# SatDump/SatDump

Measured on AMD Instinct MI355X. Metric: Msamples/s IQ through PSK demod -> Viterbi -> RS (HBM-resident cf32), higher is better.
Workload: dtype f32; 1 GPU; metop_ahrpt (BASELINE configs[2]): QPSK 2333333 sym/s @ 6 Msps cf32, conv 3/4-metop, RS(255,223) I=4, 152880 CADUs = 2146959360 samples (17.176 GB) per GPU per step; mode=chunk-parallel (speculate + certify)

## Files before the change

satdump_amd/csrc/demod_kernels.hip:

```cpp
#include "demod_kernels.h"
#include <climits>
#include <optional>
#include <type_traits>

namespace sdhip
{
    static int env_int(const char *name, int dflt)
    {
        const char *v = getenv(name);
        return (v && *v) ? atoi(v) : dflt;
    }
    struct SinCosTab
    {
        double c0, c1, c2, c3, c4, s1, s2, s3;
    };
    __device__ __forceinline__ float sd_sinf_poly(double x, double x2, bool neg_tab, int n)
    {
        const double sgn = neg_tab ? -1.0 : 1.0;
        if ((n & 1) == 0)
        {
            const double s1c = -0x1.555545995a603p-3, s2c = 0x1.1107605230bc4p-7, s3c = -0x1.994eb3774cf24p-13;
            const double x3 = x * x2;
            const double s1 = fma(x2, s3c, s2c);
            const double x7 = x3 * x2;
// ... 42 lines not shown
        if (sd_abstop12(y) < sd_abstop12(0x1.921FB6p-1f))
        {
            if (sd_abstop12(y) < sd_abstop12(0x1p-12f))
                return 1.0f;
            return sd_sinf_poly(x, x * x, false, 1);
        }
        int n;
        x = sd_reduce_fast(x, &n);
        const double sgn = ((n & 3) == 1 || (n & 3) == 2) ? -1.0 : 1.0;
        return sd_sinf_poly(x * sgn, x * x, (n & 2) != 0, n ^ 1);
    }

    __device__ __forceinline__ void sd_sincosf(float y, float &sn, float &cs)
    {
        const double x0 = (double)y;
        int n;
        const double xr = sd_reduce_fast(x0, &n);
        const double xs = ((n + 1) & 2) ? -xr : xr;
        const double x2 = xr * xr;
        const double s1c = -0x1.555545995a603p-3, s2c = 0x1.1107605230bc4p-7, s3c = -0x1.994eb3774cf24p-13;
        const double x3 = xs * x2;
        const double s1 = fma(x2, s3c, s2c);
        const double x7 = x3 * x2;
        const double sp = fma(x7, s1, fma(x3, s1c, xs));
        const double c1c = -0x1.ffffffd0c621cp-2, c2c = 0x1.55553e1068f19p-5, c3c = -0x1.6c087e89a359dp-10, c4c = 0x1.99343027bf8c3p-16;
        const double x4 = x2 * x2;
        const double c2 = fma(x2, c4c, c3c);
        const double c1 = fma(x2, c1c, 0x1p0);
        const double x6 = x4 * x2;
        const double cp0 = fma(x6, c2, fma(x4, c2c, c1));
        const float fs = (float)sp, fc0 = (float)cp0;
        const float fc = (n & 2) ? -fc0 : fc0;
        const bool odd = (n & 1) != 0;
        const bool tiny = sd_abstop12(y) < sd_abstop12(0x1p-12f);
        sn = tiny ? y : (odd ? fc : fs);
        cs = tiny ? 1.0f : (odd ? fs : fc);
    }

    __device__ __forceinline__ void sd_sincosf_fast(float y, float &sn, float &cs)
    {
        const float k = rintf(y * 0.63661977236758134308f);
        float r = fmaf(-k, 1.57079637050628662109375f, y);
        r = fmaf(-k, -4.37113900018624283e-8f, r);
        const float r2 = r * r;
        const float sp = fmaf(r2, fmaf(r2, fmaf(r2, 2.75573192239858906526e-6f, -1.98412698412698412698e-4f), 8.33333333333333333333e-3f), -1.66666666666666666667e-1f);
        const float s = fmaf(r * r2, sp, r);
        const float cp = fmaf(r2, fmaf(r2, fmaf(r2, 2.48015873015873015873e-5f, -1.38888888888888888889e-3f), 4.16666666666666666667e-2f), -0.5f);
        const float c = fmaf(r2, cp, 1.0f);
        const int q = (int)k & 3;
        const float a = (q & 1) ? c : s, b = (q & 1) ? s : c;
        sn = (q & 2) ? -a : a;
        cs = ((q + 1) & 2) ? -b : b;
    }
    __device__ __forceinline__ float sd_sqrt_fast(float x)
    {
#ifdef SDHIP_HOST_TWIN
        return sqrtf(x);
#else
        return __builtin_amdgcn_sqrtf(x);
#endif
    }
    __device__ __forceinline__ float sd_clip_med3(float x, float lo, float hi)
    {
#ifdef SDHIP_HOST_TWIN
        return x != x ? lo : x < lo ? lo : (x > hi ? hi : x);
#else
        return __builtin_amdgcn_fmed3f(x, lo, hi);
#endif
    }

    __global__ __launch_bounds__(256) void k_convert(const void *in, int fmt, int iq_swap, long long n, cf32 *out)
    {
        const long long i = (long long)blockIdx.x * blockDim.x + threadIdx.x;
        if (i >= n)
            return;
        float re, im;
        if (fmt == 0)
        {
            const cf32 v = ((const cf32 *)in)[i];
            re = v.re;
            im = v.im;
        }
        else if (fmt == 1)
        {
            const short2 v = ((const short2 *)in)[i];
            const float s = 1.0f / 32767.0f;
            re = (float)v.x * s;
            im = (float)v.y * s;
        }
        else if (fmt == 2)
        {
            const char2 v = ((const char2 *)in)[i];
            const float s = 1.0f / 127.0f;
            re = (float)v.x * s;
            im = (float)v.y * s;
        }
        else if (fmt == 3)
        {
            const uchar2 v = ((const uchar2 *)in)[i];
            re = (float)((double)((int)v.x - 127) * (1.0 / 127.0));
            im = (float)((double)((int)v.y - 127) * (1.0 / 127.0));
        }
        else
        {
            const int2 v = ((const int2 *)in)[i];
            const float sc = 1.0f / 2147483647.0f;
// ... 564 lines not shown
            int z = 0;
            asm volatile("" : "+s"(z));
#pragma unroll
            for (int j = 0; j < NT; j++)
            {
                const float tk = rtaps[z + j];
                const v2f tt{tk, tk};
#pragma unroll
                for (int r = 0; r < FIRW_R; r++)
                {
                    const v2f prod = s[r + j] * tt;
                    acc[r] = acc[r] + prod;
                }
            }
#pragma unroll
            for (int r = 0; r < FIRW_R; r++)
                tile[t * FIRW_R + r] = acc[r];
            __syncthreads();
            const long long i0 = blk * OUTS;
            for (int i = t; i < OUTS; i += FIRW_BLOCK)
                if (i0 + i < n)
                    reinterpret_cast<v2f *>(y)[i0 + i] = tile[i];
            __syncthreads();
        }
    }
    static bool fir_window_enabled()
    {
        static const bool on = [] {
            const char *e = getenv("SDHIP_FIR_WINDOW");
            return !(e && e[0] == '0');
        }();
        return on;
    }
    void launch_fir(const cf32 *x, cf32 *y, long long n, const float *rtaps_dev, int ntaps, hipStream_t st)
    {
        if (n <= 0)
            return;
        if (ntaps == 31 && fir_window_enabled())
        {
            ProfScope _ps("k_fir_window", st);
            const long long ntiles = (n + FIRW_BLOCK * FIRW_R - 1) / (FIRW_BLOCK * FIRW_R);
            static const int grid = resident_grid(k_fir_window<31>, FIRW_BLOCK);
            hipLaunchKernelGGL((k_fir_window<31>), dim3((unsigned)(ntiles < grid ? ntiles : grid)), dim3(FIRW_BLOCK), 0, st, x, y, n, rtaps_dev, ntiles);
            return;
        }
        ProfScope _ps("k_fir", st);
        hipLaunchKernelGGL(k_fir, dim3((unsigned)((n + FIR_BLOCK * FIR_PER - 1) / (FIR_BLOCK * FIR_PER))), dim3(FIR_BLOCK), 0, st, x, y, n, rtaps_dev, ntaps);
    }

    struct Blk8
    {
        float4 a, b, c, d;
    };
    template <int D, bool FASTQ = false>
    struct AgcStageT
    {
        using P = AgcParams;
        using S = AgcState;
        static constexpr int DEPTH = D;
        __device__ static __forceinline__ S init(const P &p, int k) { return S{p.starts ? p.starts[k] : p.init_gain}; }
        __device__ static __forceinline__ bool close(const S &a, const S &b, float tol_a, float) { return fabsf(a.gain - b.gain) <= tol_a * fabsf(b.gain); }
        __device__ static __forceinline__ void prewarm(S &, const P &, const cf32 *, long long) {}
        __device__ static __forceinline__ cf32 step(S &s, const P &p, const cf32 v) { return step_t<FASTQ>(s, p, v); }
        template <bool FAST>
        __device__ static __forceinline__ cf32 step_t(S &s, const P &p, const cf32 v)
        {
            const float ore = v.re * s.gain;
            const float oim = v.im * s.gain;
            float mag;
            if (p.input_mag)
            {
                float mi;
                if constexpr (FAST)
                    mi = sd_sqrt_fast(fmaf(v.re, v.re, v.im * v.im));
                else
                    mi = sqrtf(v.re * v.re + v.im * v.im);
                mag = mi * s.gain;
            }
            else if constexpr (FAST)
                mag = sd_sqrt_fast(fmaf(ore, ore, oim * oim));
            else
                mag = sqrtf(ore * ore + oim * oim) ;
            s.gain = s.gain + p.rate * (p.reference - mag);
            if (p.max_gain > 0.0f && s.gain > p.max_gain)
                s.gain = p.max_gain;
            return cf32{ore, oim};
        }
    };

    using AgcStage = AgcStageT<4>;

    __device__ __forceinline__ float sd_to_vgpr(float v)
    {
        float r;
        asm("v_mov_b32 %0, %1" : "=v"(r) : "s"(v));
        return r;
    }
    template <bool FAST>
    struct AgcFirStageT
    {
        using P = AgcFirParams;
        using S = AgcFirState;
        static constexpr int DEPTH = 4;
        static constexpr int NT = AGCFIR_NT;
        __device__ static __forceinline__ S init(const P &p, int)
        {
            S s;
            s.gain = p.agc.init_gain;
#pragma unroll
            for (int i = 0; i < 4; i++)
                s.lag[i] = p.agc.init_gain;
#pragma unroll
            for (int i = 0; i < 2 * (NT - 1); i++)
                s.w[i] = 0.0f;
            return s;
        }
        __device__ static __forceinline__ bool close(const S &a, const S &b, float tol_a, float) { return fabsf(a.gain - b.gain) <= tol_a * fabsf(b.gain); }
        __device__ static __forceinline__ void prewarm(S &, const P &, const cf32 *, long long) {}
        __device__ static __forceinline__ v2f agc(S &s, const P &p, float re, float im)
        {
            AgcState a{s.gain};
            const cf32 o = AgcStageT<4>::template step_t<FAST>(a, p.agc, cf32{re, im});
            s.gain = a.gain;
            return v2f{o.re, o.im};
        }
        __device__ static __forceinline__ Blk8 block(S &s, const P &p, const Blk8 &c, bool write)
        {
            v2f loc[NT - 1 + 8];
#pragma unroll
            for (int i = 0; i < NT - 1; i++)
                loc[i] = v2f{s.w[2 * i], s.w[2 * i + 1]};
            const float g_in = s.gain;
            loc[NT - 1 + 0] = agc(s, p, c.a.x, c.a.y);
            loc[NT - 1 + 1] = agc(s, p, c.a.z, c.a.w);
            loc[NT - 1 + 2] = agc(s, p, c.b.x, c.b.y);
            loc[NT - 1 + 3] = agc(s, p, c.b.z, c.b.w);
            loc[NT - 1 + 4] = agc(s, p, c.c.x, c.c.y);
            loc[NT - 1 + 5] = agc(s, p, c.c.z, c.c.w);
            loc[NT - 1 + 6] = agc(s, p, c.d.x, c.d.y);
            loc[NT - 1 + 7] = agc(s, p, c.d.z, c.d.w);
            Blk8 o{};
            if (write)
            {
                v2f acc[8];
#pragma unroll
                for (int r = 0; r < 8; r++)
                    acc[r] = v2f{0.0f, 0.0f};
#pragma unroll
                for (int j = 0; j < NT; j++)
                {
                    const v2f tp{sd_to_vgpr(p.taps[j & ~1]), sd_to_vgpr(p.taps[j | 1])};
                    const v2f tt = (j & 1) ? __builtin_shufflevector(tp, tp, 1, 1) : __builtin_shufflevector(tp, tp, 0, 0);
                    if constexpr (FAST)
                    {
#pragma unroll
                        for (int r = 0; r < 8; r++)
                            acc[r] = __builtin_elementwise_fma(loc[r + j], tt, acc[r]);
                    }
                    else
                    {
                        v2f prod[8];
#pragma unroll
                        for (int r = 0; r < 8; r++)
                            prod[r] = loc[r + j] * tt;
#pragma unroll
                        for (int r = 0; r < 8; r++)
                            acc[r] = acc[r] + prod[r];
                    }
                }
                o = Blk8{make_float4(acc[0].x, acc[0].y, acc[1].x, acc[1].y), make_float4(acc[2].x, acc[2].y, acc[3].x, acc[3].y),
                         make_float4(acc[4].x, acc[4].y, acc[5].x, acc[5].y), make_float4(acc[6].x, acc[6].y, acc[7].x, acc[7].y)};
            }
#pragma unroll
            for (int i = 0; i < NT - 1; i++)
            {
                s.w[2 * i] = loc[i + 8].x;
                s.w[2 * i + 1] = loc[i + 8].y;
            }
            s.lag[3] = s.lag[2];
            s.lag[2] = s.lag[1];
            s.lag[1] = s.lag[0];
            s.lag[0] = g_in;
            return o;
        }
        __device__ static __forceinline__ cf32 step(S &s, const P &p, const cf32 v)
        {
            const v2f a = agc(s, p, v.re, v.im);
            v2f acc{0.0f, 0.0f};
#pragma unroll
            for (int j = 0; j < NT - 1; j++)
            {
                const v2f prod = v2f{s.w[2 * j], s.w[2 * j + 1]} * v2f{p.taps[j], p.taps[j]};
                acc = acc + prod;
            }
            {
                const v2f prod = a * v2f{p.taps[NT - 1], p.taps[NT - 1]};
                acc = acc + prod;
            }
#pragma unroll
            for (int i = 0; i < NT - 2; i++)
            {
                s.w[2 * i] = s.w[2 * i + 2];
                s.w[2 * i + 1] = s.w[2 * i + 3];
            }
            s.w[2 * (NT - 2)] = a.x;
            s.w[2 * (NT - 2) + 1] = a.y;
            return cf32{acc.x, acc.y};
        }
    };
    using AgcFirStage = AgcFirStageT<false>;

    template <int ORDER, int D = 4, bool FAST = false, bool BCLIP = false>
    struct CostasStage
    {
        using P = CostasParams;
        using S = CostasState;
        static constexpr int DEPTH = D;
        __device__ static __forceinline__ S init(const P &p, int) { return S{0.0f, p.init_freq}; }
        __device__ static __forceinline__ bool close(const S &a, const S &b, float tol_phase, float tol_freq)
        {
            const float twopi = 6.28318530717958647692f;
            float d = a.phase - b.phase;
            d -= twopi * rintf(d / twopi);
            return fabsf(d) < tol_phase && fabsf(a.freq - b.freq) < tol_freq;
        }
        __device__ static __forceinline__ void prewarm(S &s, const P &p, const cf32 *x, long long i0)
        {
            if (p.est_len <= 0 || p.order > 4)
                return;
            const int M = p.order;
            float rc, rs;
            __sincosf(-(float)M * s.freq, &rs, &rc);
            float cr = 1.0f, ci = 0.0f, ar = 0.0f, ai = 0.0f;
            for (int n = 0; n < p.est_len; n++)
            {
                const cf32 v = x[i0 + n];
                float zr = v.re * v.re - v.im * v.im, zi = 2.0f * v.re * v.im;
                if (M == 4)
                {
                    const float tr = zr * zr - zi * zi, ti = 2.0f * zr * zi;
                    zr = tr;
                    zi = ti;
                }
                ar += zr * cr - zi * ci;
                ai += zr * ci + zi * cr;
                const float nr = cr * rc - ci * rs, ni = cr * rs + ci * rc;
                cr = nr;
                ci = ni;
            }
            const float ang = (M == 4) ? atan2f(-ai, -ar) : atan2f(ai, ar);
            s.phase = ang / (float)M;
        }
        __device__ static __forceinline__ cf32 step(S &s, const P &p, const cf32 v)
        {
            float cs, sn;
            if constexpr (FAST)
                sd_sincosf_fast(-s.phase, sn, cs);
            else
                sd_sincosf(-s.phase, sn, cs);
            const float tr = (v.re * cs) - (v.im * sn);
            const float ti = (v.im * cs) + (v.re * sn);
            float error;
            if constexpr (ORDER == 2)
                error = tr * ti;
            else if constexpr (ORDER == 4)
                error = (tr > 0.0f ? 1.0f : -1.0f) * ti - (ti > 0.0f ? 1.0f : -1.0f) * tr;
            else
            {
                const float K = sqrtf(2.0f) - 1.0f;
                const float st = tr > 0.0f ? 1.0f : -1.0f, su = ti > 0.0f ? 1.0f : -1.0f;
                const float ea = st * ti - su * tr * K, eb = st * ti * K - su * tr;
                error = fabsf(tr) >= fabsf(ti) ? ea : eb;
            }
            if constexpr (BCLIP)
                error = error < -1.0f ? -1.0f : (error > 1.0f ? 1.0f : error);
            else
                error = 0.5f * (fabsf(error + 1.0f) - fabsf(error - 1.0f));
            s.freq = s.freq + p.beta * error;
            s.phase = s.phase + (s.freq + p.alpha * error);
            const double twopi = 2 * 3.14159265358979323846;
            {
                const float twopi_f = 6.28318548202514648f;
                const double step = s.phase >= twopi_f ? -twopi : (s.phase <= -twopi_f ? twopi : 0.0);
                s.phase = (float)((double)s.phase + step);
            }
            s.freq = __builtin_fmaxf(__builtin_fminf(s.freq, p.fmax), p.fmin);
            return cf32{tr, ti};
        }
    };

    __device__ __forceinline__ float sd_fast_atan2f(float y, float x, const float *__restrict__ tab)
    {
        const float ya = fabsf(y), xa = fabsf(x);
        if (!(ya > 0.0f || xa > 0.0f))
            return 0.0f;
        const bool flat = ya < xa;
        const float z = flat ? ya / xa : xa / ya;
        float base = z;
        if (!((double)z < 0.003921569))
        {
            const float al = z * 255.0f;
            const int idx = ((int)al) & 0xff;
            const float lo = tab[idx], hi = tab[idx + 1];
            base = lo + (hi - lo) * (al - (float)idx);
        }
        const float pi = (float)3.14159265358979323846, half = (float)1.57079632679489661923;
        if (xa > ya)
            return x >= 0.0f ? (y >= 0.0f ? base : -base) : (y >= 0.0f ? pi - base : base - pi);
        return y >= 0.0f ? (x >= 0.0f ? half - base : half + base) : (x >= 0.0f ? -half + base : -half - base);
    }
    __device__ __forceinline__ float sd_fast_cos(float x)
    {
        const float x2 = x * x, x4 = x2 * x2, x8 = x4 * x4;
        return (float)((-2.7236370439787708e-7 * x2 + 2.4799852696610628e-5) * x8 + (-1.3888885054799695e-3 * x2 + 4.1666666636943683e-2) * x4 +
                       (-4.9999999999963024e-1 * x2 + 1.0000000000000000e+0));
    }
    __device__ __forceinline__ float sd_fast_sin(float x)
    {
        const float x2 = x * x, x4 = x2 * x2;
        return (float)(((2.7181216275479732e-6 * x2 - 1.9839312269456257e-4) * x4 + (8.3333293048425631e-3 * x2 - 1.6666666640797048e-1)) * x2 * x + x);
    }
    __device__ __forceinline__ float sd_wrap_pi(float v)
    {
        const double pi = 3.14159265358979323846, twopi = 2 * 3.14159265358979323846;
        while ((double)v < -pi)
            v = (float)((double)v + twopi);
        while ((double)v > pi)
            v = (float)((double)v - twopi);
        return v;
    }
    struct PllStage
    {
        using P = PllParams;
        using S = CostasState;
        static constexpr int DEPTH = 2;
        __device__ static __forceinline__ S init(const P &p, int) { return S{0.0f, p.init_freq}; }
// ... 100 lines not shown
                s.fre_im *= inv;
                s.margin = fminf(s.margin, fminf(p.fmax - s.freq, s.freq - p.fmin));
                if (s.freq > p.fmax)
                {
                    s.freq = p.fmax;
                    s.fre_re = p.lim_min_re;
                    s.fre_im = p.lim_min_im;
                }
                if (s.freq < p.fmin)
                {
                    s.freq = p.fmin;
                    s.fre_re = p.lim_max_re;
                    s.fre_im = p.lim_max_im;
                }
            }
            return cf32{tr, ti};
        }
    };

    struct DcStage
    {
        using P = DcParams;
        using S = DcState;
        static constexpr int DEPTH = 4;
        __device__ static __forceinline__ S init(const P &p, int k) { return p.starts[k]; }
        __device__ static __forceinline__ bool close(const S &a, const S &b, float tol, float)
        {
            const float m = fmaxf(fabsf(b.acc_re), fabsf(b.acc_im));
            return fabsf(a.acc_re - b.acc_re) <= tol * m && fabsf(a.acc_im - b.acc_im) <= tol * m;
        }
        __device__ static __forceinline__ void prewarm(S &, const P &, const cf32 *, long long) {}
        __device__ static __forceinline__ cf32 step(S &s, const P &, const cf32 v)
        {
            const float alpha = 0.0001f, beta = 1.0f - 0.0001f;
            s.acc_re = s.acc_re * beta + v.re * alpha;
            s.acc_im = s.acc_im * beta + v.im * alpha;
            return cf32{v.re - s.acc_re, v.im - s.acc_im};
        }
    };

    __device__ __forceinline__ Blk8 blk_load(const cf32 *x, long long i)
    {
        const float4 *xp = reinterpret_cast<const float4 *>(x + i);
        return Blk8{xp[0], xp[1], xp[2], xp[3]};
    }
    template <class Stage, class = void>
    struct stage_is_blockwise : std::false_type
    {
    };
    template <class Stage>
    struct stage_is_blockwise<Stage, std::void_t<decltype(&Stage::block)>> : std::true_type
    {
    };
    template <class Stage>
    __device__ __forceinline__ Blk8 blk_step(typename Stage::S &s, const typename Stage::P &p, const Blk8 &c, bool write)
    {
        if constexpr (stage_is_blockwise<Stage>::value)
            return Stage::block(s, p, c, write);
        else
        {
            const cf32 a0 = Stage::step(s, p, cf32{c.a.x, c.a.y});
            const cf32 a1 = Stage::step(s, p, cf32{c.a.z, c.a.w});
            const cf32 a2 = Stage::step(s, p, cf32{c.b.x, c.b.y});
            const cf32 a3 = Stage::step(s, p, cf32{c.b.z, c.b.w});
            const cf32 a4 = Stage::step(s, p, cf32{c.c.x, c.c.y});
            const cf32 a5 = Stage::step(s, p, cf32{c.c.z, c.c.w});
            const cf32 a6 = Stage::step(s, p, cf32{c.d.x, c.d.y});
            const cf32 a7 = Stage::step(s, p, cf32{c.d.z, c.d.w});
            return Blk8{make_float4(a0.re, a0.im, a1.re, a1.im), make_float4(a2.re, a2.im, a3.re, a3.im), make_float4(a4.re, a4.im, a5.re, a5.im),
                        make_float4(a6.re, a6.im, a7.re, a7.im)};
        }
    }
    template <class Stage, int D>
    __device__ __forceinline__ void group_run(typename Stage::S &s, const typename Stage::P &p, const Blk8 (&q)[D], cf32 *y, long long i, bool write)
    {
        Blk8 o[D];
#pragma unroll
        for (int d = 0; d < D; d++)
            o[d] = blk_step<Stage>(s, p, q[d], write);
        if (write)
        {
            float4 *yp = reinterpret_cast<float4 *>(y + i);
#pragma unroll
            for (int d = 0; d < D; d++)
            {
                yp[4 * d + 0] = o[d].a;
                yp[4 * d + 1] = o[d].b;
                yp[4 * d + 2] = o[d].c;
                yp[4 * d + 3] = o[d].d;
            }
        }
    }
    struct NoHook
    {
        __device__ __forceinline__ bool operator()(long long) const { return false; }
    };
    template <class Stage, bool HOOK = false, class Hook = NoHook>
    __device__ __forceinline__ void run_range(typename Stage::S &s, const typename Stage::P &p, const cf32 *x, cf32 *y, long long i0, long long i1, bool write,
                                              long long hb = 0, int hstep = 0, Hook hook = Hook())
    {
        constexpr int D = Stage::DEPTH;
        long long i = i0;
        for (; i < i1 && (i & 7); i++)
        {
            const cf32 o = Stage::step(s, p, x[i]);
            if (write)
                y[i] = o;
        }
        if (i + 8 * D <= i1)
        {
            Blk8 qa[D], qb[D];
#pragma unroll
            for (int d = 0; d < D; d++)
                qa[d] = blk_load(x, i + 8 * d);
            for (;;)
            {
                const bool more_b = i + 16 * D <= i1;
                if (more_b)
                {
#pragma unroll
                    for (int d = 0; d < D; d++)
                        qb[d] = blk_load(x, i + 8 * (D + d));
                }
                group_run<Stage, D>(s, p, qa, y, i, write);
// ... 88 lines not shown
        return b;
    }
    __device__ __forceinline__ void coop_unpack(const Burst &b, const Coop &co, Blk8 &q0, Blk8 &q1)
    {
        __builtin_amdgcn_sched_barrier(0);
        *reinterpret_cast<float4 *>(co.lw + 0 * 8 * COOP_REGION) = b.c0;
        *reinterpret_cast<float4 *>(co.lw + 1 * 8 * COOP_REGION) = b.c1;
        *reinterpret_cast<float4 *>(co.lw + 2 * 8 * COOP_REGION) = b.c2;
        *reinterpret_cast<float4 *>(co.lw + 3 * 8 * COOP_REGION) = b.c3;
        *reinterpret_cast<float4 *>(co.lw + 4 * 8 * COOP_REGION) = b.c4;
        *reinterpret_cast<float4 *>(co.lw + 5 * 8 * COOP_REGION) = b.c5;
        *reinterpret_cast<float4 *>(co.lw + 6 * 8 * COOP_REGION) = b.c6;
        *reinterpret_cast<float4 *>(co.lw + 7 * 8 * COOP_REGION) = b.c7;
        sd_wave_sync();
        const float4 *r = reinterpret_cast<const float4 *>(co.lr);
        q0 = Blk8{r[0], r[1], r[2], r[3]};
        q1 = Blk8{r[4], r[5], r[6], r[7]};
        sd_wave_sync();
        __builtin_amdgcn_sched_barrier(0);
    }
    __device__ __forceinline__ void coop_store_half(const Blk8 &o, int half, const Coop &co)
    {
        float4 *w = reinterpret_cast<float4 *>(co.sw + half * 64);
        w[0] = o.a;
        w[1] = o.b;
        w[2] = o.c;
        w[3] = o.d;
    }
    __device__ __forceinline__ void coop_store_flush(cf32 *y, long long i0w, const Coop &co)
    {
        __builtin_amdgcn_sched_barrier(0);
        sd_wave_sync();
        char *sb = reinterpret_cast<char *>(y + i0w);
#pragma unroll
        for (int j = 0; j < 8; j++)
            *reinterpret_cast<float4 *>(sb + (long long)(8 * j) * co.stride + co.voff) = *reinterpret_cast<const float4 *>(co.sr + j * 8 * COOP_REGION);
        sd_wave_sync();
        __builtin_amdgcn_sched_barrier(0);
    }
    template <class Stage, bool COOP = false, class Hook>
    __device__ __forceinline__ void run_range1(typename Stage::S &s, const typename Stage::P &p, const cf32 *x, cf32 *y, long long i0, long long i1,
                                               long long write_from, long long hb, int hstep, Hook hook, const Coop *co = nullptr)
    {
        static_assert(Stage::DEPTH == 4, "four-block groups");
        long long i = i0;
        for (; i < i1 && (i & 7); i++)
        {
            const cf32 o = Stage::step(s, p, x[i]);
            if (i >= write_from)
                y[i] = o;
        }
        if (i + 32 <= i1)
        {
            if constexpr (COOP)
            {
                const long long lim = 1ll << 30;
                const long long wf = write_from - i, tl = i1 - i;
                const int total = sd_uniform((int)(tl < lim ? tl : lim));
                const int wfrom = sd_uniform((int)(wf < -lim ? -lim : (wf < lim ? wf : lim)));
                const int hoff = sd_uniform((int)((i - hb) & (long long)(hstep - 1)));
                const long long iw = sd_uniform(i);
                const long long ibase = i;
                int r = 0;
                Burst b0 = coop_load(x, iw, *co), b1 = coop_load(x, iw + 16, *co);
                Blk8 q[4];
                for (;;)
                {
                    const bool more = r + 64 <= total;
                    const bool wr = r >= wfrom;
                    coop_unpack(b0, *co, q[0], q[1]);
#pragma unroll
                    for (int d = 0; d < 2; d++)
                    {
                        const Blk8 o = blk_step<Stage>(s, p, q[d], wr);
                        if (wr)
                            coop_store_half(o, d, *co);
                    }
                    if (wr)
                        coop_store_flush(y, iw + r, *co);
                    if (more)
                        b0 = coop_load(x, iw + r + 32, *co);
                    coop_unpack(b1, *co, q[2], q[3]);
#pragma unroll
                    for (int d = 2; d < 4; d++)
                    {
                        const Blk8 o = blk_step<Stage>(s, p, q[d], wr);
                        if (wr)
                            coop_store_half(o, d - 2, *co);
                    }
                    if (wr)
                        coop_store_flush(y, iw + r + 16, *co);
                    if (more)
                        b1 = coop_load(x, iw + r + 48, *co);
                    r += 32;
                    if ((((r + hoff) & (hstep - 1)) == 0) && r < total)
                        (void)hook(ibase + r);
                    if (!more)
                        break;
                }
                i = ibase + r;
            }
            else
            {
            Blk8 q[4];
#pragma unroll
            for (int d = 0; d < 4; d++)
                q[d] = blk_load(x, i + 8 * d);
            for (;;)
            {
                const bool more = i + 64 <= i1;
                const bool wr = i >= write_from;
#pragma unroll
                for (int d = 0; d < 4; d++)
                {
                    const Blk8 o = blk_step<Stage>(s, p, q[d], wr);
                    if (wr)
                        blk_store<Stage>(y, i + 8 * d, o);
                    if ((d & 1) && more)
                    {
                        q[d - 1] = blk_load(x, i + 32 + 8 * (d - 1));
                        q[d] = blk_load(x, i + 32 + 8 * d);
                    }
                }
                i += 32;
                if ((((i - hb) & (long long)(hstep - 1)) == 0) && i < i1 && hook(i))
                    return;
                if (!more)
                    break;
            }
            }
        }
        for (; i < i1; i++)
        {
            const cf32 o = Stage::step(s, p, x[i]);
            if (i >= write_from)
                y[i] = o;
        }
    }

    template <class Stage, bool CKPT>
    __global__ __launch_bounds__(64) void k_chunks(const cf32 *x, cf32 *y, ChunkGeom g, typename Stage::P p, const typename Stage::S *start0,
                                                   typename Stage::S *spec, typename Stage::S *endst, const int *redo, int nredo, typename Stage::S *ck,
                                                   int ck_per_chunk, int ck_len, float tol_a, float tol_b, unsigned long long *ck_work)
    {
        const int idx = (int)(blockIdx.x * blockDim.x + threadIdx.x);
        int k;
        typename Stage::S s;
        if (redo)
        {
            if (idx >= nredo)
                return;
            k = redo[idx];
            s = spec[k];
        }
        else
        {
            k = idx;
            if (k >= g.K)
                return;
            if (k == 0)
                s = *start0;
            else
            {
                s = Stage::init(p, k);
                const long long b = chunk_begin(g, k);
                Stage::prewarm(s, p, x, b - g.W);
                run_range<Stage>(s, p, x, y, b - g.W, b, false);
                spec[k] = s;
            }
        }
        const long long b = chunk_begin(g, k), e = chunk_end(g, k);
        if constexpr (!CKPT)
        {
            run_range<Stage>(s, p, x, y, b, e, true);
            endst[k] = s;
        }
        else
        {
            bool merged = false;
            int jmax = 0;
            typename Stage::S *cks = ck + (size_t)k * ck_per_chunk;
            run_range<Stage, true>(s, p, x, y, b, e, true, b, ck_len, [&](long long i) -> bool {
                const int j = (int)((i - b) / ck_len) - 1;
                if (j < 0 || j >= ck_per_chunk)
                    return false;
                jmax = j + 1;
                if (redo && Stage::close(s, cks[j], tol_a, tol_b))
                {
                    merged = true;
                    return true;
                }
                cks[j] = s;
                return false;
            });
            if (!merged)
                endst[k] = s;
            if (redo && ck_work)
            {
                atomicAdd(ck_work, 1ull);
                atomicAdd(ck_work + 1, (unsigned long long)(jmax + 1));
                atomicAdd(ck_work + 2, (unsigned long long)((e - b + ck_len - 1) / ck_len));
            }
        }
    }

    template <bool FAST>
    struct AfcAgcOnly
    {
        using P = AfcParams;
        using S = AfcState;
        static constexpr int DEPTH = 4;
        __device__ static __forceinline__ Blk8 block(S &s, const P &p, const Blk8 &c, bool) { return AgcFirStageT<FAST>::block(s.af, p.af, c, false); }
        __device__ static __forceinline__ cf32 step(S &s, const P &p, const cf32 v) { return AgcFirStageT<FAST>::step(s.af, p.af, v); }
    };
    struct AfcEstState
    {
        AfcState s;
        float cr, ci, ar, ai, rc, rs;
    };
    template <int M, bool FAST>
    struct AfcEst
    {
        using P = AfcParams;
        using S = AfcEstState;
        static constexpr int DEPTH = 4;
        __device__ static __forceinline__ void acc(S &e, float re, float im)
        {
            float zr = re * re - im * im, zi = 2.0f * re * im;
            if constexpr (M == 4)
            {
                const float tr = zr * zr - zi * zi, ti = 2.0f * zr * zi;
                zr = tr;
                zi = ti;
            }
            e.ar += zr * e.cr - zi * e.ci;
            e.ai += zr * e.ci + zi * e.cr;
            const float nr = e.cr * e.rc - e.ci * e.rs, ni = e.cr * e.rs + e.ci * e.rc;
            e.cr = nr;
            e.ci = ni;
        }
        __device__ static __forceinline__ Blk8 block(S &e, const P &p, const Blk8 &c, bool)
        {
            const Blk8 f = AgcFirStageT<FAST>::block(e.s.af, p.af, c, true);
            acc(e, f.a.x, f.a.y);
            acc(e, f.a.z, f.a.w);
            acc(e, f.b.x, f.b.y);
            acc(e, f.b.z, f.b.w);
            acc(e, f.c.x, f.c.y);
            acc(e, f.c.z, f.c.w);
            acc(e, f.d.x, f.d.y);
            acc(e, f.d.z, f.d.w);
            return f;
        }
        __device__ static __forceinline__ cf32 step(S &e, const P &p, const cf32 v)
        {
            const cf32 f = AgcFirStageT<FAST>::step(e.s.af, p.af, v);
            acc(e, f.re, f.im);
            return f;
        }
    };
    template <int ORDER, bool FAST>
    struct AfcFull
    {
        using P = AfcParams;
        using S = AfcState;
        using Cos = CostasStage<ORDER, 4, FAST>;
        static constexpr int DEPTH = 4;
        __device__ static __forceinline__ Blk8 block(S &s, const P &p, const Blk8 &c, bool)
        {
            const Blk8 f = AgcFirStageT<FAST>::block(s.af, p.af, c, true);
            const cf32 a0 = Cos::step(s.cos, p.cos, cf32{f.a.x, f.a.y});
            const cf32 a1 = Cos::step(s.cos, p.cos, cf32{f.a.z, f.a.w});
            const cf32 a2 = Cos::step(s.cos, p.cos, cf32{f.b.x, f.b.y});
            const cf32 a3 = Cos::step(s.cos, p.cos, cf32{f.b.z, f.b.w});
            const cf32 a4 = Cos::step(s.cos, p.cos, cf32{f.c.x, f.c.y});
            const cf32 a5 = Cos::step(s.cos, p.cos, cf32{f.c.z, f.c.w});
            const cf32 a6 = Cos::step(s.cos, p.cos, cf32{f.d.x, f.d.y});
            const cf32 a7 = Cos::step(s.cos, p.cos, cf32{f.d.z, f.d.w});
            return Blk8{make_float4(a0.re, a0.im, a1.re, a1.im), make_float4(a2.re, a2.im, a3.re, a3.im), make_float4(a4.re, a4.im, a5.re, a5.im),
                        make_float4(a6.re, a6.im, a7.re, a7.im)};
        }
        __device__ static __forceinline__ cf32 step(S &s, const P &p, const cf32 v) { return Cos::step(s.cos, p.cos, AgcFirStageT<FAST>::step(s.af, p.af, v)); }
    };
    __device__ __forceinline__ float sd_wrap_2pi(double ph)
    {
        const double twopi = 2 * 3.14159265358979323846;
        while (ph > twopi)
            ph -= twopi;
        while (ph < -twopi)
            ph += twopi;
        return (float)ph;
    }
    template <int ORDER, bool FAST>
    __global__ __launch_bounds__(64) __attribute__((amdgpu_waves_per_eu(2, 2))) void k_afc(const cf32 *x, cf32 *y, ChunkGeom g, AfcParams p, const AfcState *start0, AfcState *spec, AfcState *endst,
                                                const int *redo, int nredo, AfcCkpt *ck, int ck_per_chunk, int ck_len, float tol_phase, float tol_freq, int coop_nb)
    {
        __shared__ __attribute__((aligned(16))) char coop_lds[2 * COOP_LDS_BYTES];
        const int idx = (int)(blockIdx.x * blockDim.x + threadIdx.x);
        const bool coop = !redo && coop_nb > 0 && (int)blockIdx.x < coop_nb;
        const Coop co = coop_make(coop_lds, (long long)g.L * (long long)sizeof(cf32));
        int k;
        AfcState s;
        bool leave_spec = false;
        long long i0;
        if (redo)
        {
            if (idx >= nredo)
                return;
            k = redo[idx];
            s = spec[k];
            i0 = chunk_begin(g, k);
        }
        else
        {
            if (coop_nb > 0)
            {
                if (coop)
                    k = 1 + idx;
                else
                {
                    const int j = ((int)blockIdx.x - coop_nb) * 8 + (int)threadIdx.x;
                    if ((int)threadIdx.x >= 8 || j >= g.K - 64 * coop_nb)
                        return;
                    k = j == 0 ? 0 : 64 * coop_nb + j;
                }
            }
            else
            {
                k = idx;
                if (k >= g.K)
                    return;
            }
            i0 = 0;
            s = *start0;
            const long long b = chunk_begin(g, k);
            const long long w0 = b - g.W - p.w_agc;
            if (k > 0)
                leave_spec = true;
            if (k > 0 && w0 > 0)
            {
                const auto nohook = [](long long) { return false; };
                const long long never = 1ll << 62;
                s.af = AgcFirStage::init(p.af, k);
                s.cos = CostasState{0.0f, p.cos.init_freq};
                if (coop)
                    run_range1<AfcAgcOnly<FAST>, true>(s, p, x, y, w0, b - g.W, never, 0, 1 << 30, nohook, &co);
                else
                    run_range1<AfcAgcOnly<FAST>>(s, p, x, y, w0, b - g.W, never, 0, 1 << 30, nohook);
                i0 = b - g.W;
                if (p.cos.est_len > 0 && ORDER <= 4)
                {
                    constexpr int M = ORDER <= 2 ? 2 : 4;
                    AfcEstState e;
                    e.s = s;
                    __sincosf(-(float)M * s.cos.freq, &e.rs, &e.rc);
                    e.cr = 1.0f;
                    e.ci = 0.0f;
                    e.ar = 0.0f;
                    e.ai = 0.0f;
                    if (coop)
                        run_range1<AfcEst<M, FAST>, true>(e, p, x, y, i0, i0 + p.cos.est_len, never, 0, 1 << 30, nohook, &co);
                    else
                        run_range1<AfcEst<M, FAST>>(e, p, x, y, i0, i0 + p.cos.est_len, never, 0, 1 << 30, nohook);
                    s = e.s;
                    const float ang = (M == 4) ? atan2f(-e.ai, -e.ar) : atan2f(e.ai, e.ar);
                    s.cos.phase = sd_wrap_2pi((double)(ang / (float)M) + (double)s.cos.freq * (double)p.cos.est_len);
                    i0 += p.cos.est_len;
                }
            }
        }
        const long long b = chunk_begin(g, k), e = chunk_end(g, k);
        bool merged = false;
        AfcCkpt *cks = ck ? ck + (size_t)k * ck_per_chunk : nullptr;
        const auto hook = [&](long long i) -> bool {
            if (i < b)
                return false;
            if (i == b)
            {
                if (leave_spec)
                    spec[k] = s;
                return false;
            }
            const int j = (int)((i - b) / ck_len) - 1;
            if (!cks || j >= ck_per_chunk)
                return false;
            if (redo)
            {
                const AfcCkpt o = cks[j];
                if (__float_as_uint(o.gain) == __float_as_uint(s.af.gain) && __float_as_uint(o.lag3) == __float_as_uint(s.af.lag[3]) &&
                    CostasStage<ORDER, 4>::close(s.cos, CostasState{o.phase, o.freq}, tol_phase, tol_freq))
                {
                    merged = true;
                    return true;
                }
            }
            cks[j] = AfcCkpt{s.af.gain, s.af.lag[3], s.cos.phase, s.cos.freq};
            return false;
        };
        if (coop)
            run_range1<AfcFull<ORDER, FAST>, true>(s, p, x, y, i0, e, b, b, ck_len, hook, &co);
        else
            run_range1<AfcFull<ORDER, FAST>>(s, p, x, y, i0, e, b, b, ck_len, hook);
        if (!merged)
            endst[k] = s;
    }
    void launch_afc(const cf32 *x, cf32 *y, const ChunkGeom &g, const AfcParams &p, const AfcState *start0, AfcState *spec, AfcState *endst, const int *redo,
                    int nredo, hipStream_t st, const AfcCkptCfg &ck, bool fast)
    {
        const int n = redo ? nredo : g.K;
        if (n <= 0)
            return;
        ProfScope _ps("k_afc", st);
        std::optional<ProfScope> _pr;
        if (redo)
            _pr.emplace("k_afc (re-run launches, included in k_afc)", st);
        auto go = [&](auto order, auto fm) {
            constexpr int O = decltype(order)::value;
            constexpr bool F = decltype(fm)::value;
            const bool coop_env = env_int("SDHIP_COOP", 1) != 0;
            int coop_nb = 0;
            if (coop_env && !redo && g.L % 16 == 0 && g.W % 16 == 0 && p.w_agc % 16 == 0 && p.cos.est_len % 16 == 0 && (long long)g.L > (long long)p.w_agc && g.K >= 66)
                coop_nb = (g.K - 2) / 64;
            const int nblk = coop_nb > 0 ? coop_nb + (g.K - 64 * coop_nb + 7) / 8 : (n + 63) / 64;
            if (!redo && coop_nb == 0 && g.K >= 66 && getenv("SDHIP_COOP_REQUIRE"))
                throw HipError("k_afc: cooperative access asked for (SDHIP_COOP_REQUIRE) but the geometry does not allow it");
            if (getenv("SDHIP_DEBUG") && !redo)
                fprintf(stderr, "[sdhip] k_afc: K %d L %d W %d w_agc %d est %d -> %d cooperative blocks of %d\n", g.K, g.L, g.W, p.w_agc, p.cos.est_len, coop_nb, nblk);
            hipLaunchKernelGGL((k_afc<O, F>), dim3(nblk), dim3(64), 0, st, x, y, g, p, start0, spec, endst, redo, nredo, ck.ck, ck.per_chunk,
                               ck.len > 0 ? ck.len : 2048, ck.tol_phase, ck.tol_freq, coop_nb);
        };
        auto by_order = [&](auto fm) {
            if (p.cos.order == 2)
                go(std::integral_constant<int, 2>{}, fm);
            else if (p.cos.order == 4)
                go(std::integral_constant<int, 4>{}, fm);
            else
                go(std::integral_constant<int, 8>{}, fm);
        };
        if (fast)
            by_order(std::true_type{});
        else
            by_order(std::false_type{});
    }

    __global__ __launch_bounds__(256) void k_dc_partial(const cf32 *x, ChunkGeom g, double *partial)
    {
        __shared__ double sr[256], si[256];
        const int k = (int)blockIdx.x, t = (int)threadIdx.x;
        const long long b = chunk_begin(g, k), e = chunk_end(g, k);
        const double beta = (double)(1.0f - 0.0001f), alpha = (double)0.0001f;
        const double up = pow(beta, -256.0);
        double ar = 0, ai = 0;
        if (b + t < e)
        {
            double w = pow(beta, (double)(e - 1 - (b + t))) * alpha;
            for (long long i = b + t; i < e; i += 256)
            {
                const cf32 v = x[i];
                ar += w * (double)v.re;
                ai += w * (double)v.im;
                w *= up;
            }
        }
        sr[t] = ar;
        si[t] = ai;
        __syncthreads();
        for (int s2 = 128; s2 > 0; s2 >>= 1)
        {
            if (t < s2)
            {
                sr[t] += sr[t + s2];
                si[t] += si[t + s2];
            }
            __syncthreads();
        }
        if (t == 0)
        {
            partial[2 * k] = sr[0];
            partial[2 * k + 1] = si[0];
        }
    }
    struct AgcMap
    {
        double a, b, c;
    };
    __device__ __forceinline__ AgcMap agc_map_then(const AgcMap &f1, const AgcMap &f2)
    {
        return AgcMap{f2.a * f1.a, f2.a * f1.b + f2.b, fmin(f2.a * f1.c + f2.b, f2.c)};
    }
    constexpr int AGCP_TILE = 2048;
    __global__ __launch_bounds__(256) void k_agc_partial(const cf32 *x, ChunkGeom g, AgcParams p, double *partial)
    {
        __shared__ float mag[AGCP_TILE];
        __shared__ double sa[256], sb[256], sc[256];
        __shared__ int bad;
// ... 1360 lines not shown
```

Measured before the change: 55500 Msamples/s.

## Specialize AFC kernel on AGC flags and software-pipeline FIR taps with Costas

Adds a compile-time AGC flag variant of k_afc, so the input_mag and max_gain branches fold away when max_gain is set and input_mag is off. For that variant, the AGC+FIR stage splits the 31-tap convolution into a carry of early taps computed one block ahead, interleaved with the serial Costas loop using sched barriers. It also adds a branchless sincos sign flip and phase wrap. The intent is to hide the Costas dependency chain behind FIR arithmetic, at the cost of more registers (waves_per_eu fixed at 2) and more kernel instances.

```diff
diff --git a/satdump_amd/csrc/demod_kernels.hip b/satdump_amd/csrc/demod_kernels.hip
--- a/satdump_amd/csrc/demod_kernels.hip
+++ b/satdump_amd/csrc/demod_kernels.hip
@@ -118,6 +118,22 @@
         sn = (q & 2) ? -a : a;
         cs = ((q + 1) & 2) ? -b : b;
     }
+    __device__ __forceinline__ void sd_sincosf_fast_sb(float y, float &sn, float &cs)
+    {
+        const float k = rintf(y * 0.63661977236758134308f);
+        float r = fmaf(-k, 1.57079637050628662109375f, y);
+        r = fmaf(-k, -4.37113900018624283e-8f, r);
+        const float r2 = r * r;
+        const float sp = fmaf(r2, fmaf(r2, fmaf(r2, 2.75573192239858906526e-6f, -1.98412698412698412698e-4f), 8.33333333333333333333e-3f), -1.66666666666666666667e-1f);
+        const float s = fmaf(r * r2, sp, r);
+        const float cp = fmaf(r2, fmaf(r2, fmaf(r2, 2.48015873015873015873e-5f, -1.38888888888888888889e-3f), 4.16666666666666666667e-2f), -0.5f);
+        const float c = fmaf(r2, cp, 1.0f);
+        const int q = (int)k;
+        const float a = (q & 1) ? c : s, b = (q & 1) ? s : c;
+        const unsigned t = (unsigned)q << 30;
+        sn = __uint_as_float(__float_as_uint(a) ^ (t & 0x80000000u));
+        cs = __uint_as_float(__float_as_uint(b) ^ ((t + 0x40000000u) & 0x80000000u));
+    }
     __device__ __forceinline__ float sd_sqrt_fast(float x)
     {
 #ifdef SDHIP_HOST_TWIN
@@ -788,6 +804,9 @@
     {
         float4 a, b, c, d;
     };
+    constexpr unsigned AFC_INPUT_MAG = 1,
+                       AFC_MAX_GAIN = 2,
+                       AFC_GENERIC = 4;
     template <int D, bool FASTQ = false>
     struct AgcStageT
     {
@@ -798,13 +817,14 @@
         __device__ static __forceinline__ bool close(const S &a, const S &b, float tol_a, float) { return fabsf(a.gain - b.gain) <= tol_a * fabsf(b.gain); }
         __device__ static __forceinline__ void prewarm(S &, const P &, const cf32 *, long long) {}
         __device__ static __forceinline__ cf32 step(S &s, const P &p, const cf32 v) { return step_t<FASTQ>(s, p, v); }
-        template <bool FAST>
+        template <bool FAST, unsigned AV = AFC_GENERIC>
         __device__ static __forceinline__ cf32 step_t(S &s, const P &p, const cf32 v)
         {
+            static_assert(AV == AFC_GENERIC || (AV & ~(AFC_INPUT_MAG | AFC_MAX_GAIN)) == 0, "AFC_GENERIC stands alone");
             const float ore = v.re * s.gain;
             const float oim = v.im * s.gain;
             float mag;
-            if (p.input_mag)
+            if ((AV & AFC_GENERIC) ? p.input_mag != 0 : (AV & AFC_INPUT_MAG) != 0)
             {
                 float mi;
                 if constexpr (FAST)
@@ -818,7 +838,7 @@
             else
                 mag = sqrtf(ore * ore + oim * oim) ;
             s.gain = s.gain + p.rate * (p.reference - mag);
-            if (p.max_gain > 0.0f && s.gain > p.max_gain)
+            if (((AV & AFC_GENERIC) ? p.max_gain > 0.0f : (AV & AFC_MAX_GAIN) != 0) && s.gain > p.max_gain)
                 s.gain = p.max_gain;
             return cf32{ore, oim};
         }
@@ -832,7 +852,13 @@
         asm("v_mov_b32 %0, %1" : "=v"(r) : "s"(v));
         return r;
     }
-    template <bool FAST>
+    __device__ __forceinline__ void sd_pin(v2f &v)
+    {
+#ifndef SDHIP_HOST_TWIN
+        asm volatile("" : "+v"(v));
+#endif
+    }
+    template <bool FAST, unsigned AV = AFC_GENERIC>
     struct AgcFirStageT
     {
         using P = AgcFirParams;
@@ -856,7 +882,7 @@
         __device__ static __forceinline__ v2f agc(S &s, const P &p, float re, float im)
         {
             AgcState a{s.gain};
-            const cf32 o = AgcStageT<4>::template step_t<FAST>(a, p.agc, cf32{re, im});
+            const cf32 o = AgcStageT<4>::template step_t<FAST, AV>(a, p.agc, cf32{re, im});
             s.gain = a.gain;
             return v2f{o.re, o.im};
         }
@@ -919,6 +945,99 @@
             s.lag[0] = g_in;
             return o;
         }
+        struct Carry
+        {
+            v2f acc[8];
+        };
+        __device__ static __forceinline__ void taps_range(v2f (&acc)[8], const v2f *win, const P &p, const int j0, const int j1, const int lo, const int hi)
+        {
+#pragma unroll
+            for (int j = 0; j < NT; j++)
+            {
+                if (j < j0 || j > j1)
+                    continue;
+                const v2f tp{sd_to_vgpr(p.taps[j & ~1]), sd_to_vgpr(p.taps[j | 1])};
+                const v2f tt = (j & 1) ? __builtin_shufflevector(tp, tp, 1, 1) : __builtin_shufflevector(tp, tp, 0, 0);
+#pragma unroll
+                for (int r = 0; r < 8; r++)
+                {
+                    if (j < lo - r || j > hi - r)
+                        continue;
+                    if constexpr (FAST)
+                        acc[r] = __builtin_elementwise_fma(win[r + j], tt, acc[r]);
+                    else
+                    {
+                        const v2f prod = win[r + j] * tt;
+                        acc[r] = acc[r] + prod;
+                    }
+                }
+            }
+        }
+        __device__ static __forceinline__ void early_taps(Carry &k, const v2f *win, const P &p)
+        {
+#pragma unroll
+            for (int r = 0; r < 8; r++)
+                k.acc[r] = v2f{0.0f, 0.0f};
+            taps_range(k.acc, win, p, 0, NT - 2, 0, NT - 2);
+        }
+        __device__ static __forceinline__ void prime(const S &s, const P &p, Carry &k)
+        {
+            v2f win[NT - 1];
+#pragma unroll
+            for (int i = 0; i < NT - 1; i++)
+                win[i] = v2f{s.w[2 * i], s.w[2 * i + 1]};
+            early_taps(k, win, p);
+        }
+        template <class Sink>
+        __device__ static __forceinline__ Blk8 block_pipe(S &s, const P &p, const Blk8 &c, Carry &k, Sink &&sink)
+        {
+            v2f loc[NT - 1 + 8];
+#pragma unroll
+            for (int i = 0; i < NT - 1; i++)
+                loc[i] = v2f{s.w[2 * i], s.w[2 * i + 1]};
+            const float g_in = s.gain;
+            __builtin_amdgcn_sched_barrier(0);
+            loc[NT - 1 + 0] = agc(s, p, c.a.x, c.a.y);
+            loc[NT - 1 + 1] = agc(s, p, c.a.z, c.a.w);
+            loc[NT - 1 + 2] = agc(s, p, c.b.x, c.b.y);
+            loc[NT - 1 + 3] = agc(s, p, c.b.z, c.b.w);
+            loc[NT - 1 + 4] = agc(s, p, c.c.x, c.c.y);
+            loc[NT - 1 + 5] = agc(s, p, c.c.z, c.c.w);
+            loc[NT - 1 + 6] = agc(s, p, c.d.x, c.d.y);
+            loc[NT - 1 + 7] = agc(s, p, c.d.z, c.d.w);
+            v2f f[8];
+#pragma unroll
+            for (int r = 0; r < 8; r++)
+                f[r] = k.acc[r];
+            taps_range(f, loc, p, NT - 1 - 7, NT - 1, NT - 1, NT - 1 + 7);
+            __builtin_amdgcn_sched_barrier(0);
+#pragma unroll
+            for (int r = 0; r < 8; r++)
+                k.acc[r] = v2f{0.0f, 0.0f};
+            cf32 o[8];
+#pragma unroll
+            for (int r = 0; r < 8; r++)
+            {
+                taps_range(k.acc, loc + 8, p, 4 * r, 4 * r + 3, 0, NT - 2);
+                o[r] = sink(cf32{f[r].x, f[r].y});
+#pragma unroll
+                for (int q = 0; q < 8; q++)
+                    sd_pin(k.acc[q]);
+                __builtin_amdgcn_sched_barrier(0);
+            }
+#pragma unroll
+            for (int i = 0; i < NT - 1; i++)
+            {
+                s.w[2 * i] = loc[i + 8].x;
+                s.w[2 * i + 1] = loc[i + 8].y;
+            }
+            s.lag[3] = s.lag[2];
+            s.lag[2] = s.lag[1];
+            s.lag[1] = s.lag[0];
+            s.lag[0] = g_in;
+            return Blk8{make_float4(o[0].re, o[0].im, o[1].re, o[1].im), make_float4(o[2].re, o[2].im, o[3].re, o[3].im), make_float4(o[4].re, o[4].im, o[5].re, o[5].im),
+                        make_float4(o[6].re, o[6].im, o[7].re, o[7].im)};
+        }
         __device__ static __forceinline__ cf32 step(S &s, const P &p, const cf32 v)
         {
             const v2f a = agc(s, p, v.re, v.im);
@@ -946,7 +1065,7 @@
     };
     using AgcFirStage = AgcFirStageT<false>;
 
-    template <int ORDER, int D = 4, bool FAST = false, bool BCLIP = false>
+    template <int ORDER, int D = 4, bool FAST = false, bool BCLIP = false, bool TRIM = false>
     struct CostasStage
     {
         using P = CostasParams;
@@ -990,7 +1109,9 @@
         __device__ static __forceinline__ cf32 step(S &s, const P &p, const cf32 v)
         {
             float cs, sn;
-            if constexpr (FAST)
+            if constexpr (FAST && TRIM)
+                sd_sincosf_fast_sb(-s.phase, sn, cs);
+            else if constexpr (FAST)
                 sd_sincosf_fast(-s.phase, sn, cs);
             else
                 sd_sincosf(-s.phase, sn, cs);
@@ -1017,7 +1138,15 @@
             const double twopi = 2 * 3.14159265358979323846;
             {
                 const float twopi_f = 6.28318548202514648f;
-                const double step = s.phase >= twopi_f ? -twopi : (s.phase <= -twopi_f ? twopi : 0.0);
+                double step;
+                if constexpr (TRIM)
+                {
+                    const bool out = fabsf(s.phase) >= twopi_f;
+                    const unsigned hi = 0x401921FBu | (~__float_as_uint(s.phase) & 0x80000000u);
+                    step = __builtin_bit_cast(double, ((unsigned long long)(out ? hi : 0u) << 32) | (unsigned long long)(out ? 0x54442D18u : 0u));
+                }
+                else
+                    step = s.phase >= twopi_f ? -twopi : (s.phase <= -twopi_f ? twopi : 0.0);
                 s.phase = (float)((double)s.phase + step);
             }
             s.freq = __builtin_fmaxf(__builtin_fminf(s.freq, p.fmax), p.fmin);
@@ -1224,6 +1353,19 @@
     struct stage_is_blockwise<Stage, std::void_t<decltype(&Stage::block)>> : std::true_type
     {
     };
+    struct NoCarry
+    {
+    };
+    template <class Stage, class = void>
+    struct stage_carry
+    {
+        using type = NoCarry;
+    };
+    template <class Stage>
+    struct stage_carry<Stage, std::void_t<typename Stage::Carry>>
+    {
+        using type = typename Stage::Carry;
+    };
     template <class Stage>
     __device__ __forceinline__ Blk8 blk_step(typename Stage::S &s, const typename Stage::P &p, const Blk8 &c, bool write)
     {
@@ -1242,6 +1384,14 @@
             return Blk8{make_float4(a0.re, a0.im, a1.re, a1.im), make_float4(a2.re, a2.im, a3.re, a3.im), make_float4(a4.re, a4.im, a5.re, a5.im),
                         make_float4(a6.re, a6.im, a7.re, a7.im)};
         }
+    }
+    template <class Stage>
+    __device__ __forceinline__ Blk8 blk_step(typename Stage::S &s, const typename Stage::P &p, const Blk8 &c, bool write, typename stage_carry<Stage>::type &k)
+    {
+        if constexpr (!std::is_same<typename stage_carry<Stage>::type, NoCarry>::value)
+            return Stage::block_carry(s, p, c, k);
+        else
+            return blk_step<Stage>(s, p, c, write);
     }
     template <class Stage, int D>
     __device__ __forceinline__ void group_run(typename Stage::S &s, const typename Stage::P &p, const Blk8 (&q)[D], cf32 *y, long long i, bool write)
@@ -1436,6 +1586,9 @@
         }
         if (i + 32 <= i1)
         {
+            typename stage_carry<Stage>::type carry;
+            if constexpr (!std::is_same<typename stage_carry<Stage>::type, NoCarry>::value)
+                Stage::prime(s, p, carry);
             if constexpr (COOP)
             {
                 const long long lim = 1ll << 30;
@@ -1456,7 +1609,7 @@
 #pragma unroll
                     for (int d = 0; d < 2; d++)
                     {
-                        const Blk8 o = blk_step<Stage>(s, p, q[d], wr);
+                        const Blk8 o = blk_step<Stage>(s, p, q[d], wr, carry);
                         if (wr)
                             coop_store_half(o, d, *co);
                     }
@@ -1468,7 +1621,7 @@
 #pragma unroll
                     for (int d = 2; d < 4; d++)
                     {
-                        const Blk8 o = blk_step<Stage>(s, p, q[d], wr);
+                        const Blk8 o = blk_step<Stage>(s, p, q[d], wr, carry);
                         if (wr)
                             coop_store_half(o, d - 2, *co);
                     }
@@ -1497,7 +1650,7 @@
 #pragma unroll
                 for (int d = 0; d < 4; d++)
                 {
-                    const Blk8 o = blk_step<Stage>(s, p, q[d], wr);
+                    const Blk8 o = blk_step<Stage>(s, p, q[d], wr, carry);
                     if (wr)
                         blk_store<Stage>(y, i + 8 * d, o);
                     if ((d & 1) && more)
@@ -1588,21 +1741,21 @@
         }
     }
 
-    template <bool FAST>
+    template <bool FAST, unsigned AV>
     struct AfcAgcOnly
     {
         using P = AfcParams;
         using S = AfcState;
         static constexpr int DEPTH = 4;
-        __device__ static __forceinline__ Blk8 block(S &s, const P &p, const Blk8 &c, bool) { return AgcFirStageT<FAST>::block(s.af, p.af, c, false); }
-        __device__ static __forceinline__ cf32 step(S &s, const P &p, const cf32 v) { return AgcFirStageT<FAST>::step(s.af, p.af, v); }
+        __device__ static __forceinline__ Blk8 block(S &s, const P &p, const Blk8 &c, bool) { return AgcFirStageT<FAST, AV>::block(s.af, p.af, c, false); }
+        __device__ static __forceinline__ cf32 step(S &s, const P &p, const cf32 v) { return AgcFirStageT<FAST, AV>::step(s.af, p.af, v); }
     };
     struct AfcEstState
     {
         AfcState s;
         float cr, ci, ar, ai, rc, rs;
     };
-    template <int M, bool FAST>
+    template <int M, bool FAST, unsigned AV>
     struct AfcEst
     {
         using P = AfcParams;
@@ -1625,7 +1778,7 @@
         }
         __device__ static __forceinline__ Blk8 block(S &e, const P &p, const Blk8 &c, bool)
         {
-            const Blk8 f = AgcFirStageT<FAST>::block(e.s.af, p.af, c, true);
+            const Blk8 f = AgcFirStageT<FAST, AV>::block(e.s.af, p.af, c, true);
             acc(e, f.a.x, f.a.y);
             acc(e, f.a.z, f.a.w);
             acc(e, f.b.x, f.b.y);
@@ -1638,21 +1791,32 @@
         }
         __device__ static __forceinline__ cf32 step(S &e, const P &p, const cf32 v)
         {
-            const cf32 f = AgcFirStageT<FAST>::step(e.s.af, p.af, v);
+            const cf32 f = AgcFirStageT<FAST, AV>::step(e.s.af, p.af, v);
             acc(e, f.re, f.im);
             return f;
         }
     };
-    template <int ORDER, bool FAST>
+    template <int ORDER, bool FAST, unsigned AV>
     struct AfcFull
     {
         using P = AfcParams;
         using S = AfcState;
-        using Cos = CostasStage<ORDER, 4, FAST>;
+        static constexpr bool SPEC = AV != AFC_GENERIC;
+        using Cos = CostasStage<ORDER, 4, FAST, false, SPEC>;
+        using AF = AgcFirStageT<FAST, AV>;
+#ifndef SDHIP_AFC_PIPE
+#define SDHIP_AFC_PIPE 1
+#endif
+        using Carry = std::conditional_t<SPEC && SDHIP_AFC_PIPE, typename AF::Carry, NoCarry>;
         static constexpr int DEPTH = 4;
+        __device__ static __forceinline__ void prime(const S &s, const P &p, Carry &k) { AF::prime(s.af, p.af, k); }
+        __device__ static __forceinline__ Blk8 block_carry(S &s, const P &p, const Blk8 &c, Carry &k)
+        {
+            return AF::block_pipe(s.af, p.af, c, k, [&](const cf32 v) { return Cos::step(s.cos, p.cos, v); });
+        }
         __device__ static __forceinline__ Blk8 block(S &s, const P &p, const Blk8 &c, bool)
         {
-            const Blk8 f = AgcFirStageT<FAST>::block(s.af, p.af, c, true);
+            const Blk8 f = AgcFirStageT<FAST, AV>::block(s.af, p.af, c, true);
             const cf32 a0 = Cos::step(s.cos, p.cos, cf32{f.a.x, f.a.y});
             const cf32 a1 = Cos::step(s.cos, p.cos, cf32{f.a.z, f.a.w});
             const cf32 a2 = Cos::step(s.cos, p.cos, cf32{f.b.x, f.b.y});
@@ -1664,7 +1828,7 @@
             return Blk8{make_float4(a0.re, a0.im, a1.re, a1.im), make_float4(a2.re, a2.im, a3.re, a3.im), make_float4(a4.re, a4.im, a5.re, a5.im),
                         make_float4(a6.re, a6.im, a7.re, a7.im)};
         }
-        __device__ static __forceinline__ cf32 step(S &s, const P &p, const cf32 v) { return Cos::step(s.cos, p.cos, AgcFirStageT<FAST>::step(s.af, p.af, v)); }
+        __device__ static __forceinline__ cf32 step(S &s, const P &p, const cf32 v) { return Cos::step(s.cos, p.cos, AgcFirStageT<FAST, AV>::step(s.af, p.af, v)); }
     };
     __device__ __forceinline__ float sd_wrap_2pi(double ph)
     {
@@ -1675,10 +1839,11 @@
             ph += twopi;
         return (float)ph;
     }
-    template <int ORDER, bool FAST>
+    template <int ORDER, bool FAST, unsigned AV>
     __global__ __launch_bounds__(64) __attribute__((amdgpu_waves_per_eu(2, 2))) void k_afc(const cf32 *x, cf32 *y, ChunkGeom g, AfcParams p, const AfcState *start0, AfcState *spec, AfcState *endst,
                                                 const int *redo, int nredo, AfcCkpt *ck, int ck_per_chunk, int ck_len, float tol_phase, float tol_freq, int coop_nb)
     {
+        static_assert(AV == AFC_GENERIC || AV == AFC_MAX_GAIN, "k_afc: the generic instance, or the one flag word the engine can hand it (no input_mag, max_gain on)");
         __shared__ __attribute__((aligned(16))) char coop_lds[2 * COOP_LDS_BYTES];
         const int idx = (int)(blockIdx.x * blockDim.x + threadIdx.x);
         const bool coop = !redo && coop_nb > 0 && (int)blockIdx.x < coop_nb;
@@ -1728,9 +1893,9 @@
                 s.af = AgcFirStage::init(p.af, k);
                 s.cos = CostasState{0.0f, p.cos.init_freq};
                 if (coop)
-                    run_range1<AfcAgcOnly<FAST>, true>(s, p, x, y, w0, b - g.W, never, 0, 1 << 30, nohook, &co);
+                    run_range1<AfcAgcOnly<FAST, AV>, true>(s, p, x, y, w0, b - g.W, never, 0, 1 << 30, nohook, &co);
                 else
-                    run_range1<AfcAgcOnly<FAST>>(s, p, x, y, w0, b - g.W, never, 0, 1 << 30, nohook);
+                    run_range1<AfcAgcOnly<FAST, AV>>(s, p, x, y, w0, b - g.W, never, 0, 1 << 30, nohook);
                 i0 = b - g.W;
                 if (p.cos.est_len > 0 && ORDER <= 4)
                 {
@@ -1743,9 +1908,9 @@
                     e.ar = 0.0f;
                     e.ai = 0.0f;
                     if (coop)
-                        run_range1<AfcEst<M, FAST>, true>(e, p, x, y, i0, i0 + p.cos.est_len, never, 0, 1 << 30, nohook, &co);
+                        run_range1<AfcEst<M, FAST, AV>, true>(e, p, x, y, i0, i0 + p.cos.est_len, never, 0, 1 << 30, nohook, &co);
                     else
-                        run_range1<AfcEst<M, FAST>>(e, p, x, y, i0, i0 + p.cos.est_len, never, 0, 1 << 30, nohook);
+                        run_range1<AfcEst<M, FAST, AV>>(e, p, x, y, i0, i0 + p.cos.est_len, never, 0, 1 << 30, nohook);
                     s = e.s;
                     const float ang = (M == 4) ? atan2f(-e.ai, -e.ar) : atan2f(e.ai, e.ar);
                     s.cos.phase = sd_wrap_2pi((double)(ang / (float)M) + (double)s.cos.freq * (double)p.cos.est_len);
@@ -1782,9 +1947,9 @@
             return false;
         };
         if (coop)
-            run_range1<AfcFull<ORDER, FAST>, true>(s, p, x, y, i0, e, b, b, ck_len, hook, &co);
+            run_range1<AfcFull<ORDER, FAST, AV>, true>(s, p, x, y, i0, e, b, b, ck_len, hook, &co);
         else
-            run_range1<AfcFull<ORDER, FAST>>(s, p, x, y, i0, e, b, b, ck_len, hook);
+            run_range1<AfcFull<ORDER, FAST, AV>>(s, p, x, y, i0, e, b, b, ck_len, hook);
         if (!merged)
             endst[k] = s;
     }
@@ -1798,33 +1963,46 @@
         std::optional<ProfScope> _pr;
         if (redo)
             _pr.emplace("k_afc (re-run launches, included in k_afc)", st);
-        auto go = [&](auto order, auto fm) {
-            constexpr int O = decltype(order)::value;
-            constexpr bool F = decltype(fm)::value;
-            const bool coop_env = env_int("SDHIP_COOP", 1) != 0;
-            int coop_nb = 0;
-            if (coop_env && !redo && g.L % 16 == 0 && g.W % 16 == 0 && p.w_agc % 16 == 0 && p.cos.est_len % 16 == 0 && (long long)g.L > (long long)p.w_agc && g.K >= 66)
-                coop_nb = (g.K - 2) / 64;
-            const int nblk = coop_nb > 0 ? coop_nb + (g.K - 64 * coop_nb + 7) / 8 : (n + 63) / 64;
-            if (!redo && coop_nb == 0 && g.K >= 66 && getenv("SDHIP_COOP_REQUIRE"))
-                throw HipError("k_afc: cooperative access asked for (SDHIP_COOP_REQUIRE) but the geometry does not allow it");
-            if (getenv("SDHIP_DEBUG") && !redo)
-                fprintf(stderr, "[sdhip] k_afc: K %d L %d W %d w_agc %d est %d -> %d cooperative blocks of %d\n", g.K, g.L, g.W, p.w_agc, p.cos.est_len, coop_nb, nblk);
-            hipLaunchKernelGGL((k_afc<O, F>), dim3(nblk), dim3(64), 0, st, x, y, g, p, start0, spec, endst, redo, nredo, ck.ck, ck.per_chunk,
-                               ck.len > 0 ? ck.len : 2048, ck.tol_phase, ck.tol_freq, coop_nb);
+        const int spec_sw = env_int("SDHIP_AFC_SPEC", 1);
+        if (spec_sw != 0 && spec_sw != 1)
+            throw HipError("SDHIP_AFC_SPEC: 0 or 1");
+        if (p.cos.order != 2 && p.cos.order != 4 && p.cos.order != 8)
+            throw HipError("k_afc: Costas order 2, 4 or 8");
+        const unsigned av_exact = (p.af.agc.input_mag ? AFC_INPUT_MAG : 0u) | (p.af.agc.max_gain > 0.0f ? AFC_MAX_GAIN : 0u);
+        const unsigned av = (spec_sw == 1 && av_exact == AFC_MAX_GAIN) ? AFC_MAX_GAIN : AFC_GENERIC;
+        const bool coop_env = env_int("SDHIP_COOP", 1) != 0;
+        int coop_nb = 0;
+        if (coop_env && !redo && g.L % 16 == 0 && g.W % 16 == 0 && p.w_agc % 16 == 0 && p.cos.est_len % 16 == 0 && (long long)g.L > (long long)p.w_agc && g.K >= 66)
+            coop_nb = (g.K - 2) / 64;
+        const int nblk = coop_nb > 0 ? coop_nb + (g.K - 64 * coop_nb + 7) / 8 : (n + 63) / 64;
+        if (!redo && coop_nb == 0 && g.K >= 66 && getenv("SDHIP_COOP_REQUIRE"))
+            throw HipError("k_afc: cooperative access asked for (SDHIP_COOP_REQUIRE) but the geometry does not allow it");
+        if (getenv("SDHIP_DEBUG") && !redo)
+            fprintf(stderr, "[sdhip] k_afc: K %d L %d W %d w_agc %d est %d -> %d cooperative blocks of %d, AGC flags %u\n", g.K, g.L, g.W, p.w_agc, p.cos.est_len, coop_nb, nblk, av);
+        auto go = [&](auto kern) {
+            hipLaunchKernelGGL(kern, dim3(nblk), dim3(64), 0, st, x, y, g, p, start0, spec, endst, redo, nredo, ck.ck, ck.per_chunk, ck.len > 0 ? ck.len : 2048, ck.tol_phase,
+                               ck.tol_freq, coop_nb);
         };
-        auto by_order = [&](auto fm) {
-            if (p.cos.order == 2)
-                go(std::integral_constant<int, 2>{}, fm);
-            else if (p.cos.order == 4)
-                go(std::integral_constant<int, 4>{}, fm);
-            else
-                go(std::integral_constant<int, 8>{}, fm);
-        };
-        if (fast)
-            by_order(std::true_type{});
-        else
-            by_order(std::false_type{});
+        const unsigned key = ((unsigned)p.cos.order << 8) | (fast ? 16u : 0u) | av;
+#define AFC_INSTANCE(O, F, V) case ((unsigned)(O) << 8) | ((F) ? 16u : 0u) | (V): return go(k_afc<(O), (F), (V)>);
+        switch (key)
+        {
+            AFC_INSTANCE(4, true, AFC_MAX_GAIN)
+            AFC_INSTANCE(2, true, AFC_MAX_GAIN)
+            AFC_INSTANCE(8, true, AFC_MAX_GAIN)
+            AFC_INSTANCE(4, false, AFC_MAX_GAIN)
+            AFC_INSTANCE(2, false, AFC_MAX_GAIN)
+            AFC_INSTANCE(8, false, AFC_MAX_GAIN)
+            AFC_INSTANCE(4, true, AFC_GENERIC)
+            AFC_INSTANCE(2, true, AFC_GENERIC)
+            AFC_INSTANCE(8, true, AFC_GENERIC)
+            AFC_INSTANCE(4, false, AFC_GENERIC)
+            AFC_INSTANCE(2, false, AFC_GENERIC)
+            AFC_INSTANCE(8, false, AFC_GENERIC)
+        default:
+            throw HipError("k_afc: no instance for this combination of variant flags");
+        }
+#undef AFC_INSTANCE
     }
 
     __global__ __launch_bounds__(256) void k_dc_partial(const cf32 *x, ChunkGeom g, double *partial)
```

New measurement: 53820 Msamples/s. -3.0%, worse.
